# afermg/aliby

Hardware: AMD Instinct MI355X
Metric: FOV tiles/sec (whole node) (higher is better)
Workload: dtype u16 pixels, f64 feature accumulators, f32 dynamics, bfloat16 U-Net

## Files before the change

aliby_amd/_lib.py:

```python

from __future__ import annotations

import ctypes as C
import os
import threading
from pathlib import Path

import numpy as np

_HERE = Path(__file__).resolve().parent
LIB_PATH = Path(os.environ["ALIBY_HIP_LIB"]) if os.environ.get("ALIBY_HIP_LIB") else _HERE / "libaliby_hip.so"

OK, ERR_INVALID, ERR_OVERFLOW, ERR_HIP, ERR_TOO_LARGE, ERR_UNSUPPORTED = range(6)
U16, F32 = 0, 1
U8W = 4
U64, F64 = 2, 3
RED_MAX, RED_ADD, RED_DIV = 0, 1, 2


class AlibyHipError(RuntimeError):
    pass


class aliby_object(C.Structure):
# ... 90 lines not shown
    "aliby_nn_nhwc_to_nchw_f32": (_i, [_vp, _vp, _i, _i, _i, _i, _i, _vp, _vp, _vp]),
    "aliby_nn_tiles_to_nhwc8_bf16": (_i, [_vp, _vp, _i, _i, _i, _i, _vp, _vp, _vp, _vp, _vp]),
    "aliby_masks_workspace_bytes": (_sz, [_i, _i, _i]),
    "aliby_masks_from_flows": (_i, [_vp, _vp, _vp, _i, _i, _i, _i, C.c_float, C.c_float, _i, C.c_float, _vp, _sz,
                                    _vp, _vp, _vp, _vp]),
    "aliby_masks3d_workspace_bytes": (_sz, [_i, _i, _i, _i]),
    "aliby_masks_from_flows_3d": (_i, [_vp, _vp, _vp, _i, _i, _i, _i, _i, C.c_float, _i, C.c_float, _vp, _sz, _vp, _vp, _vp, _vp]),
    "aliby_features_intensity": (_i, [_vp, _vp, _vp, _i, _i, _i, _i, _i, _i, _vp, _i, _i, _i, _vp, _i, _i, _vp]),
    "aliby_features_sizeshape": (_i, [_vp, _vp, _i, _i, _i, _vp, _i, _i, _i, _i, _vp, _i, _i, _vp]),
    "aliby_features_feret": (_i, [_vp, _vp, _i, _i, _i, _vp, _i, _i, _vp, _i, _i, _vp]),
    "aliby_object_mec": (_i, [_vp, _vp, _i, _i, _i, _vp, _i, _i, _vp, _vp]),
    "aliby_features_zernike": (_i, [_vp, _vp, _vp, _i, _i, _i, _i, _i, _i, _vp, _i, _vp, _i, _vp, _i, _i, _vp]),
    "aliby_features_radial_zernikes_multi": (_i, [_vp, _vp, _vp, _i, _i, _i, _i, _i, _vp, _vp, _i, _vp, _i, _vp, _vp, _i, _vp]),
    "aliby_features_texture": (_i, [_vp, _vp, _vp, _i, _i, _i, _i, _i, _i, _vp, _i, _i, _i, _i, _i, _i, _vp, _i, _i, _vp]),
    "aliby_radial_geometry": (_i, [_vp, _vp, _i, _i, _i, _vp, _i, _i, _i, _i, _vp, _vp]),
    "aliby_features_radial_distribution": (_i, [_vp, _vp, _vp, _vp, _i, _i, _i, _i, _i, _i, _vp, _i, _i, _vp, _i, _i, _vp]),
    "aliby_features_cell_ratio": (_i, [_vp, _vp, _vp, _i, _i, _i, _i, _i, _i, _i, _vp, _i, _i, _vp, _vp]),
    "aliby_features_trap_background": (_i, [_vp, _vp, _vp, _i, _i, _i, _i, _i, _i, _vp, _vp]),
    "aliby_granularity_workspace_bytes": (_sz, [_i, _i, _i, _i, C.c_double, C.c_double]),
    "aliby_features_granularity": (_i, [_vp, _vp, _vp, _i, _i, _i, _i, _i, _i, _vp, _i, C.c_double, C.c_double, _i, _i, _i,
                                        _vp, _sz, _vp, _i, _i, _vp]),
    "aliby_radial_geometry_unscaled": (_i, [_vp, _vp, _i, _i, _i, _vp, _i, _i, _i, _i, C.c_double, _vp, _vp]),
    "aliby_features_radial_distribution_rings": (_i, [_vp, _vp, _vp, _vp, _i, _i, _i, _i, _i, _i, _vp, _i, _i, _i, _vp, _i, _i, _vp]),
    "aliby_features_cell": (_i, [_vp, _vp, _vp, _i, _i, _i, _i, _i, _i, _vp, _i, _i, _i, _i, _vp, _i, _i, _vp]),
    "aliby_features_coloc": (_i, [_vp, _vp, _vp, _i, _i, _i, _i, _i, _i, _i, _vp, _i, _i, _vp, _i, _i, _i, _i, _i,
                                  C.c_double, C.c_double, _vp, _vp, _vp]),
    "aliby_labels_apply_lut": (_i, [_vp, _vp, _i, _i, _i, _vp, _vp, _vp, _vp]),
    "aliby_features_intensity3d": (_i, [_vp, _vp, _vp, _i, _i, _i, _i, _i, _i, _vp, _vp, _i, _i, _vp]),
    "aliby_features_sizeshape3d": (_i, [_vp, _vp, _i, _i, _i, _i, _vp, _vp, _vp, _i, _i, _vp]),
    "aliby_coloc3d_lds_voxels": (_i, []),
    "aliby_features_coloc3d": (_i, [_vp, _vp, _vp, _i, _i, _i, _i, _i, _i, _vp, _i, _vp, _vp, _i, _i, _i, _i, _i, _i, _i,
                                    C.c_double, C.c_double, _vp]),
    "aliby_texture3d_lds_voxels": (_i, []),
    "aliby_features_texture3d": (_i, [_vp, _vp, _vp, _i, _i, _i, _i, _i, _i, _i, _vp, _i, _i, _vp, _i, _i, _vp]),
    "aliby_parquet_write": (_i, [C.c_char_p, _vp, _i, _vp, _i, _vp, _vp, _i]),
    "aliby_npz_write": (_i, [C.c_char_p, _vp, _i, _i]),
    "aliby_host_codecs": (_i, [C.POINTER(_i), C.POINTER(_i)]),
    "aliby_host_copy": (_i, [_vp, _vp, _sz, _i]),
    "aliby_object_ranks": (_i, [_vp, _vp, _vp, _i, _i, _i, _i, _i, _i, _vp, _i, _i, _vp, _vp, _vp]),
}

_lib = None


def exported_symbols() -> list[str]:
    return sorted(_SIGNATURES)


def load() -> C.CDLL:
    global _lib
    if _lib is not None:
        return _lib
    if not LIB_PATH.exists():
        raise AlibyHipError(
            f"{LIB_PATH} is missing: build it with `python -c 'import __graft_entry__ as g; g.build()'` "
            "(make -C aliby_amd/csrc). There is no CPU fallback for the HIP path."
        )
    try:
        import torch
    except Exception:
        pass
    lib = C.CDLL(str(LIB_PATH), mode=getattr(os, "RTLD_NOW", 2))
# ... 80 lines not shown
```

aliby_amd/csrc/feat_coloc.hip:

```cpp
#include "common.h"
#include "coloc_stats.h"

typedef unsigned short u16;

struct ColocArgs {
  const u16* labels;
  const void* planes;
  int F, C, Y, X, ch0, ch1;
  const aliby_object* tab;
  int n_obj;
  int cap;
  unsigned char* gscratch;
  double* out;
  int ld;
  int col_pearson, col_manders, col_rwc, col_costes;
  double thr;
  double scale_max;
  const unsigned int* ranks;
  const int* rmax;
};

struct PlaneRanks {
  const unsigned int* rk1;
  const unsigned int* rk2;
// ... 273 lines not shown
        if (lane == 0) {
          const double d1 = FA ? c4[0] : 0.0, d2 = SA ? c4[1] : 0.0;
          out[col_costes] = CA ? c4[2] / d1 : 0.0;
          out[col_costes + 1] = CA ? c4[3] / d2 : 0.0;
        }
      }
    }
  }
}


struct RankArgs {
  const u16* labels;
  const void* planes;
  int F, C, Y, X, channel;
  const aliby_object* tab;
  int n_obj, cap;
  unsigned char* gscratch;
  unsigned int* ranks;
  int* rmax;
};

template <typename T, bool GLOBAL>
__global__ __launch_bounds__(256) void k_ranks(RankArgs a) {
  extern __shared__ __align__(16) unsigned char lds_raw[];
  __shared__ int wsum[4];
  __shared__ int part[256];
  unsigned char* ws = GLOBAL ? (a.gscratch + (size_t)blockIdx.x * (size_t)a.cap * 16) : lds_raw;
  float* vals = reinterpret_cast<float*>(ws);
  float* S = vals + a.cap;
  int* P = reinterpret_cast<int*>(S + a.cap);
  int* pix = P + a.cap;
  const int tid = threadIdx.x;
  const size_t plane = (size_t)a.Y * a.X;
  for (int oi = blockIdx.x; oi < a.n_obj; oi += gridDim.x) {
    const aliby_object o = a.tab[oi];
    if (o.area <= 0) { if (tid == 0) a.rmax[(size_t)oi * a.C + a.channel] = 0; continue; }
    const u16* lab = a.labels + (size_t)o.tile * plane;
    const T* px = reinterpret_cast<const T*>(a.planes) + ((size_t)o.tile * a.C + a.channel) * plane;
    unsigned int* rk = a.ranks + ((size_t)o.tile * a.C + a.channel) * plane;
    const int h = o.y1 - o.y0, w = o.x1 - o.x0, npix = h * w;
    const u16 L = (u16)o.label;
    __syncthreads();
    int base = 0;
    for (int i0 = 0; i0 < npix; i0 += blockDim.x) {
      const int i = i0 + tid;
      bool in = false;
      size_t idx = 0;
      if (i < npix) { idx = (size_t)(o.y0 + i / w) * a.X + (o.x0 + i % w); in = lab[idx] == L; }
      const int pos = block_compact_slot(in, base, wsum);
      if (in) { vals[pos] = px_load<T>(px, idx); pix[pos] = (int)idx; }
    }
    __syncthreads();
    const int N = base;
    bool done = false;
    if (sizeof(T) == 2 && !GLOBAL) {
      int lo = INT_MAX, hi = 0;
      for (int j = tid; j < N; j += blockDim.x) { const int v = (int)vals[j]; lo = min(lo, v); hi = max(hi, v); }
      const int vmin = block_min_i32(lo, part), vmax = block_max_i32(hi, part);
      const int w0 = vmin >> 5, nw = (vmax >> 5) - w0 + 1;
      if (nw <= a.cap) {
        unsigned int* bits = reinterpret_cast<unsigned int*>(S);
        __syncthreads();
        for (int i = tid; i < nw; i += blockDim.x) bits[i] = 0u;
        __syncthreads();
        for (int j = tid; j < N; j += blockDim.x) { const int v = (int)vals[j]; atomicOr(&bits[(v >> 5) - w0], 1u << (v & 31)); }
        __syncthreads();
        for (int i = tid; i < nw; i += blockDim.x) P[i] = __popc(bits[i]);
        __syncthreads();
        block_inclusive_scan(P, nw, part);
        for (int j = tid; j < N; j += blockDim.x) {
          const int v = (int)vals[j], wi = (v >> 5) - w0;
          const unsigned int below = bits[wi] & ((1u << (v & 31)) - 1u);
          rk[pix[j]] = (unsigned int)(P[wi] - __popc(bits[wi]) + __popc(below));
        }
        if (tid == 0) a.rmax[(size_t)oi * a.C + a.channel] = P[nw - 1] - 1;
        done = true;
      }
    }
    if (done) { __syncthreads(); continue; }
    const int n2 = next_pow2(N);
    for (int i = tid; i < n2; i += blockDim.x) S[i] = (i < N) ? vals[i] : INFINITY;
    block_bitonic_sort(S, n2);
    for (int i = tid; i < N; i += blockDim.x) P[i] = (i > 0 && S[i] != S[i - 1]) ? 1 : 0;
    __syncthreads();
    block_inclusive_scan(P, N, part);
    for (int j = tid; j < N; j += blockDim.x) {
      const float v = vals[j];
      int lo = 0, hi = N;
      while (lo < hi) { const int mid = (lo + hi) >> 1; if (S[mid] < v) lo = mid + 1; else hi = mid; }
      rk[pix[j]] = (unsigned int)P[lo];
    }
    if (tid == 0) a.rmax[(size_t)oi * a.C + a.channel] = P[N - 1];
    __syncthreads();
  }
}

extern "C" int aliby_object_ranks(aliby_ctx* ctx, const uint16_t* labels, const void* planes, int dtype, int F, int C,
                                  int Y, int X, int channel, const aliby_object* table_dev, int n_obj, int max_area,
                                  uint32_t* ranks_dev, int32_t* rmax_dev, void* stream) {
  ARG_CHECK(ctx != nullptr, "ctx is NULL");
  if (n_obj == 0) return ALIBY_OK;
  ARG_CHECK(labels && planes && table_dev && ranks_dev && rmax_dev, "NULL argument");
  ARG_CHECK(dtype == ALIBY_U16 || dtype == ALIBY_F32, "dtype must be ALIBY_U16 or ALIBY_F32");
  ARG_CHECK(channel >= 0 && channel < C, "channel out of range");
  ARG_CHECK((size_t)Y * X < (size_t)INT_MAX, "plane too large");
  RankArgs a;
  a.labels = labels; a.planes = planes; a.F = F; a.C = C; a.Y = Y; a.X = X; a.channel = channel; a.tab = table_dev;
  a.n_obj = n_obj; a.ranks = ranks_dev; a.rmax = rmax_dev;
  int cap = 64;
  while (cap < max_area) cap <<= 1;
  a.cap = cap;
  hipStream_t s = as_stream(stream);
  const size_t need = (size_t)cap * 16;
  if (need <= 96 * 1024) {
    a.gscratch = nullptr;
    dim3 grid(n_obj), block(aliby_pick_block(max_area));
    if (dtype == ALIBY_U16) {
      if (need > 32 * 1024) HIP_TRY(hipFuncSetAttribute((const void*)k_ranks<u16, false>, hipFuncAttributeMaxDynamicSharedMemorySize, (int)need));
      hipLaunchKernelGGL((k_ranks<u16, false>), grid, block, need, s, a);
    } else {
      if (need > 32 * 1024) HIP_TRY(hipFuncSetAttribute((const void*)k_ranks<float, false>, hipFuncAttributeMaxDynamicSharedMemorySize, (int)need));
      hipLaunchKernelGGL((k_ranks<float, false>), grid, block, need, s, a);
    }
  } else {
    const int g = n_obj < 512 ? n_obj : 512;
    int rc = aliby_ensure_scratch(ctx, (size_t)g * need);
    if (rc) return rc;
    a.gscratch = (unsigned char*)ctx->scratch;
    dim3 grid(g), block(256);
    if (dtype == ALIBY_U16) hipLaunchKernelGGL((k_ranks<u16, true>), grid, block, 0, s, a);
    else hipLaunchKernelGGL((k_ranks<float, true>), grid, block, 0, s, a);
  }
  KERNEL_CHECK();
  return ALIBY_OK;
}

extern "C" int aliby_features_coloc(aliby_ctx* ctx, const uint16_t* labels, const void* planes, int dtype,
                                    int F, int C, int Y, int X, int ch0, int ch1,
                                    const aliby_object* table_dev, int n_obj, int max_area,
                                    double* out, int ld, int col_pearson, int col_manders, int col_rwc,
                                    int col_costes, double thr_percent, double costes_scale_max,
                                    const uint32_t* ranks_dev, const int32_t* rmax_dev, void* stream) {
  ARG_CHECK(ctx != nullptr, "ctx is NULL");
  if (n_obj == 0) return ALIBY_OK;
  ARG_CHECK(labels && planes && table_dev && out, "NULL argument");
  ARG_CHECK(dtype == ALIBY_U16 || dtype == ALIBY_F32, "dtype must be ALIBY_U16 or ALIBY_F32");
  ARG_CHECK(ch0 >= 0 && ch0 < C && ch1 >= 0 && ch1 < C, "channel out of range");
  ARG_CHECK(F > 0 && Y > 0 && X > 0 && max_area >= 0, "bad shape");
  const int cols[4] = {col_pearson, col_manders, col_rwc, col_costes};
  for (int k = 0; k < 4; ++k) ARG_CHECK(cols[k] < 0 || cols[k] + 2 <= ld, "columns exceed row stride");
  ColocArgs a;
  a.labels = labels; a.planes = planes; a.F = F; a.C = C; a.Y = Y; a.X = X; a.ch0 = ch0; a.ch1 = ch1;
  a.tab = table_dev; a.n_obj = n_obj; a.out = out; a.ld = ld;
  a.col_pearson = col_pearson; a.col_manders = col_manders; a.col_rwc = col_rwc; a.col_costes = col_costes;
  a.thr = thr_percent; a.scale_max = costes_scale_max;
  a.ranks = ranks_dev; a.rmax = rmax_dev;
  ARG_CHECK(col_rwc < 0 || (ranks_dev && rmax_dev), "rwc needs the rank planes (aliby_object_ranks)");
// ... 86 lines not shown
```

aliby_amd/csrc/feat_radial.hip:

```cpp
#include "common.h"

typedef unsigned short u16;

#define RD_MAXBINS 16
#define RD_INF 0xFFFFu

struct RadialGeoArgs {
  const u16* labels;
  int F, Y, X;
  const aliby_object* tab;
  int n_obj;
  size_t cap_cells;
  unsigned char* gscratch;
  int bin_count;
  double max_radius;
  unsigned char* binmap;
};

__device__ __forceinline__ double path_cost(unsigned int w) {
  return (double)(w & 0xFFFFu) * 0.70710678118654752440 + (double)(w >> 16) * 1.0;
}

template <bool GLOBAL>
__global__ __launch_bounds__(256) void k_radial_geometry(RadialGeoArgs a) {
// ... 164 lines not shown
    if (tid < a.nout) {
      double T_ = 0, N_ = 0;
      for (int b = 0; b <= nb; ++b) { T_ += tot[b]; N_ += (double)cnt[b]; }
      const double fd = tot[tid] / T_;
      const double fb = (double)cnt[tid] / N_;
      double mean = 0;
      int nw = 0;
      double m8[8];
      for (int k = 0; k < 8; ++k)
        if (wcnt[tid][k] > 0) { m8[nw] = wsum[tid][k] / (double)wcnt[tid][k]; mean += m8[nw]; ++nw; }
      double cv = 0.0;
      if (nw > 0) {
        mean /= (double)nw;
        double var = 0;
        for (int k = 0; k < nw; ++k) var += (m8[k] - mean) * (m8[k] - mean);
        cv = sqrt(var / (double)nw) / mean;
      }
      out[tid] = fd;
      out[a.nout + tid] = fd / (fb + 2.220446049250313e-16);
      out[2 * a.nout + tid] = cv;
    }
    __syncthreads();
  }
}

extern "C" {

int aliby_radial_geometry(aliby_ctx* ctx, const uint16_t* labels, int F, int Y, int X,
                          const aliby_object* table_dev, int n_obj, int max_h, int max_w, int bin_count,
                          uint8_t* binmap_dev, void* stream) {
  return aliby_radial_geometry_unscaled(ctx, labels, F, Y, X, table_dev, n_obj, max_h, max_w, bin_count, 0.0, binmap_dev, stream);
}

int aliby_radial_geometry_unscaled(aliby_ctx* ctx, const uint16_t* labels, int F, int Y, int X,
                                   const aliby_object* table_dev, int n_obj, int max_h, int max_w, int bin_count,
                                   double maximum_radius, uint8_t* binmap_dev, void* stream) {
  ARG_CHECK(ctx != nullptr, "ctx is NULL");
  if (n_obj == 0) return ALIBY_OK;
  ARG_CHECK(labels && table_dev && binmap_dev, "NULL argument");
  ARG_CHECK(F > 0 && Y > 0 && X > 0 && max_h >= 0 && max_w >= 0, "bad shape");
  ARG_CHECK(bin_count >= 1 && bin_count < RD_MAXBINS, "1 <= bin_count < 16");
  ARG_CHECK(max_h + max_w < 16000, "object too large for 16-bit path counters");
  RadialGeoArgs a;
  a.labels = labels; a.F = F; a.Y = Y; a.X = X; a.tab = table_dev; a.n_obj = n_obj; a.bin_count = bin_count;
  a.max_radius = maximum_radius;
  a.binmap = binmap_dev;
// ... 28 lines not shown
                                             const void* planes, int dtype, int F, int C, int Y, int X,
                                             int channel, const aliby_object* table_dev, int n_obj,
                                             int bin_count, int rings_out, double* out, int ld, int col0, void* stream) {
  ARG_CHECK(ctx != nullptr, "ctx is NULL");
  ARG_CHECK(rings_out == bin_count || rings_out == bin_count + 1, "rings_out is bin_count (scaled) or bin_count + 1 (with the overflow ring)");
  if (n_obj == 0) return ALIBY_OK;
  ARG_CHECK(labels && binmap_dev && planes && table_dev && out, "NULL argument");
  ARG_CHECK(dtype == ALIBY_U16 || dtype == ALIBY_F32, "dtype must be ALIBY_U16 or ALIBY_F32");
  ARG_CHECK(channel >= 0 && channel < C, "channel out of range");
  ARG_CHECK(bin_count >= 1 && bin_count < RD_MAXBINS, "1 <= bin_count < 16");
  ARG_CHECK(col0 >= 0 && col0 + 3 * rings_out <= ld, "columns exceed row stride");
  RadialStatArgs a;
  a.labels = labels; a.binmap = binmap_dev; a.planes = planes; a.F = F; a.C = C; a.Y = Y; a.X = X;
  a.channel = channel; a.tab = table_dev; a.n_obj = n_obj; a.bin_count = bin_count;
  a.nout = rings_out;
  a.out = out; a.ld = ld; a.col0 = col0;
  hipStream_t s = as_stream(stream);
  if (dtype == ALIBY_U16) hipLaunchKernelGGL((k_radial_stats<u16>), dim3(n_obj), dim3(256), 0, s, a);
  else hipLaunchKernelGGL((k_radial_stats<float>), dim3(n_obj), dim3(256), 0, s, a);
  KERNEL_CHECK();
  return ALIBY_OK;
}

}
```

aliby_amd/extraction/engine.py:

```python

from __future__ import annotations

import ctypes as C
from dataclasses import dataclass

import numpy as np
import torch

from aliby_amd import _lib
from aliby_amd.extraction import features as feat


def _stream_ptr() -> int:
    return torch.cuda.current_stream().cuda_stream


def _ptr(t) -> int:
    if t is None:
        return 0
    if isinstance(t, torch.Tensor):
        return t.data_ptr()
    if isinstance(t, np.ndarray):
        return t.ctypes.data
    raise TypeError(type(t))
# ... 474 lines not shown
        with self.timed("radial_geometry"):
            _lib.check(self.lib.aliby_radial_geometry_unscaled(
                self.ctx.handle, _ptr(labels), F, Y, X, _ptr(table.dev), table.n_obj, table.max_h, table.max_w, int(bin_count),
                0.0 if maximum_radius is None else float(maximum_radius), _ptr(binmap), _stream_ptr()))
        cache[key] = binmap
        return binmap

    def radial_distribution(self, labels, planes, dtype, channel, table: ObjectTable, out, col0, bin_count=4,
                            scaled=True, maximum_radius=100):
        if not scaled and not maximum_radius > 0:
            raise ValueError("radial_distribution(scaled=False) needs maximum_radius > 0")
        F, Cn, Y, X = planes.shape
        binmap = self.radial_geometry(labels, table, bin_count, None if scaled else maximum_radius)
        rings = bin_count if scaled else bin_count + 1
        with self.timed("radial_distribution"):
            _lib.check(
                self.lib.aliby_features_radial_distribution_rings(
                    self.ctx.handle, _ptr(labels), _ptr(binmap), _ptr(planes), _kdt(dtype), F, Cn, Y, X, int(channel),
                    _ptr(table.dev), table.n_obj, int(bin_count), rings, _ptr(out), out.stride(0), col0, _stream_ptr(),
                )
            )
        return 3 * rings

    def granularity(self, labels, planes, dtype, channel, table: ObjectTable, out, col0, subsample_size=0.25,
                    image_sample_size=0.25, element_size=10, granular_spectrum_length=16, image_mask="frame", mask_order=1):
        if image_mask not in ("frame", "objects"):
            raise ValueError(f"image_mask must be 'frame' or 'objects', got {image_mask!r}")
        if image_mask == "objects" and int(mask_order) != 1:
            raise NotImplementedError("granularity(image_mask='objects') is built for mask_order=1 (bilinear) only")
        F, Cn, Y, X = planes.shape
        L = int(granular_spectrum_length)
        need = int(self.lib.aliby_granularity_workspace_bytes(F, Y, X, table.n_obj, float(subsample_size), float(image_sample_size)))
        work = torch.empty((need + 7) // 8, dtype=torch.float64, device=labels.device)
        with self.timed("granularity"):
            _lib.check(
                self.lib.aliby_features_granularity(
                    self.ctx.handle, _ptr(labels), _ptr(planes), _kdt(dtype), F, Cn, Y, X, int(channel), _ptr(table.dev), table.n_obj,
                    float(subsample_size), float(image_sample_size), int(element_size), L, 1 if image_mask == "objects" else 0,
                    _ptr(work), work.numel() * 8, _ptr(out), out.stride(0) if table.n_obj else max(L + col0, 1), col0, _stream_ptr(),
                )
            )
        return L

    CELL_COLUMNS = ("area", "centroid_x", "centroid_y", "conical_volume", "eccentricity", "spherical_volume", "volume",
                    "min_ax", "maj_ax", "mean", "median", "std", "total", "total_squared", "max2p5pc", "max5px_median",
                    "moment_of_inertia")
# ... 16 lines not shown
        F, Cn, Y, X = planes.shape
        out = torch.full((max(table.n_obj, 1),), float("nan"), dtype=torch.float64, device=labels.device)
        with self.timed("cell_metrics"):
            _lib.check(self.lib.aliby_features_cell_ratio(self.ctx.handle, _ptr(labels), _ptr(planes), _kdt(dtype), F, Cn, Y, X, int(ch0), int(ch1),
                                                          _ptr(table.dev), table.n_obj, table.max_area, _ptr(out), _stream_ptr()))
        return out[: table.n_obj]

    def trap_background(self, labels, planes, dtype, channel) -> torch.Tensor:
        F, Cn, Y, X = planes.shape
        out = torch.empty((F, 2), dtype=torch.float64, device=labels.device)
        with self.timed("trap_background"):
            _lib.check(self.lib.aliby_features_trap_background(self.ctx.handle, _ptr(labels), _ptr(planes), _kdt(dtype), F, Cn, Y, X, int(channel),
                                                               _ptr(out), _stream_ptr()))
        return out

    def rank_planes(self, labels, planes, dtype, table: ObjectTable, channels):
        F, Cn, Y, X = planes.shape
        key = ("ranks", planes.data_ptr())
        cache = table.__dict__.setdefault("_ranks", {})
        if key not in cache:
            cache[key] = dict(ranks=torch.empty((F, Cn, Y, X), dtype=torch.int32, device=planes.device),
                              rmax=torch.zeros((max(table.n_obj, 1), Cn), dtype=torch.int32, device=planes.device), done=set())
        e = cache[key]
        for ch in channels:
            if ch in e["done"]:
                continue
            with self.timed("ranks"):
                _lib.check(self.lib.aliby_object_ranks(self.ctx.handle, _ptr(labels), _ptr(planes), _kdt(dtype), F, Cn, Y, X, int(ch),
                                                       _ptr(table.dev), table.n_obj, table.max_area, _ptr(e["ranks"]),
                                                       _ptr(e["rmax"]), _stream_ptr()))
            e["done"].add(ch)
        return e["ranks"], e["rmax"]

    def coloc_pairs(self, labels, planes, dtype, pairs, table: ObjectTable, out, thr=15.0, scale_max=255.0) -> bool:
        F, Cn, Y, X = planes.shape
        chans = sorted({c for (pair, _) in pairs for c in pair})
        any_rwc = any(cols.get("rwc") is not None for _, cols in pairs)
        cap = 64
        while cap < table.max_area:
            cap <<= 1
        if len(pairs) > 28 or len(chans) > 8 or len(chans) * cap * 4 * (2 if any_rwc else 1) > 144 * 1024:
            return False
        ranks = rmax = None
        if any_rwc:
            ranks, rmax = self.rank_planes(labels, planes, dtype, table, tuple(chans))
        c = lambda cols, k: -1 if cols.get(k) is None else int(cols[k])
        spec = np.asarray([[ch0, ch1, c(cols, "pearson"), c(cols, "manders_fold"), c(cols, "rwc"), c(cols, "costes")]
                           for (ch0, ch1), cols in pairs], dtype=np.int32)
        with self.timed("coloc"):
            _lib.check(
                self.lib.aliby_features_coloc_pairs(
                    self.ctx.handle, _ptr(labels), _ptr(planes), _kdt(dtype), F, Cn, Y, X, spec.ctypes.data, len(pairs), _ptr(table.dev),
                    table.n_obj, table.max_area, _ptr(out), out.stride(0), float(thr), float(scale_max),
                    _ptr(ranks) if ranks is not None else 0, _ptr(rmax) if rmax is not None else 0, _stream_ptr(),
# ... 21 lines not shown
```

aliby_amd/extraction/families.py:

```python

from __future__ import annotations

import torch

from aliby_amd import _lib
from aliby_amd.extraction import features as feat
from aliby_amd.extraction.engine import _ptr, _stream_ptr

_RED = {"max": _lib.RED_MAX, "add": _lib.RED_ADD, "div": _lib.RED_DIV}


class PlaneCache:

    def __init__(self, eng, planes):
        self.eng = eng
        self.tensor, self.dtype = planes
        if self.tensor.ndim != 5:
            raise Exception(f"pixels must be [F,C,Z,Y,X], got {tuple(self.tensor.shape)}")
        self._cache = {}

    def get(self, red_z):
        if red_z in self._cache:
            return self._cache[red_z]
        if red_z not in _RED:
# ... 203 lines not shown
        for inst, reg, kw, col0, _ in specs:
            (ch0, ch1), red_ch, red_z, metric = inst[0], inst[1], inst[2], inst[3]
            if red_ch != "None":
                raise NotImplementedError(
                    "channel-combining multi instructions (extract.py:227-235) are not built; "
                    "the builder only emits red_ch='None' (pipe_builder.py:33-43)"
                )
            thr = float(kw.get("thr", 15.0)) if metric in ("manders_fold", "rwc") else None
            scale_max = float(kw.get("scale_max", 255.0)) if metric == "costes" else None
            groups.setdefault(((ch0, ch1), red_z), []).append((metric, col0, thr, scale_max))
        split = {}
        for key, entries in groups.items():
            thrs = sorted({t for _, _, t, _ in entries if t is not None})
            scale_max = next((sm for _, _, _, sm in entries if sm is not None), 255.0)
            if len(thrs) <= 1:
                split[(key, 0)] = dict(cols={m: c for m, c, _, _ in entries}, thr=thrs[0] if thrs else 15.0, scale_max=scale_max)
            else:
                for k, t in enumerate(thrs):
                    cols = {m: c for m, c, tt, _ in entries if tt == t or (tt is None and k == 0)}
                    split[(key, k)] = dict(cols=cols, thr=t, scale_max=scale_max)
        groups = {(pair_z, k): g for (pair_z, k), g in split.items()}
        if cache is None:
            raise Exception("pixels are required for colocalisation instructions")
        for (((ch0, ch1), red_z), _k), g in groups.items():
            plane, dt = cache.get(red_z)
            if "rwc" in g["cols"]:
                eng.rank_planes(labels, plane, dt, table, (ch0, ch1))
        import os

        batches = {}
        for (((ch0, ch1), red_z), _k), g in groups.items():
            batches.setdefault((red_z, g["thr"], g["scale_max"]), []).append(((ch0, ch1), g["cols"]))
        left = []
        for (red_z, thr, scale_max), pairs in batches.items():
            plane, dt = cache.get(red_z)
            if os.environ.get("ALIBY_COLOC_PAIRS", "1") == "0" or len(pairs) < 2 or not eng.coloc_pairs(
                    labels, plane, dt, pairs, table, out, thr=thr, scale_max=scale_max):
                left.extend((pair, red_z, cols, thr, scale_max) for pair, cols in pairs)
        if left:
            fan.fork()
            for (ch0, ch1), red_z, cols, thr, scale_max in left:
                plane, dt = cache.get(red_z)
                with fan.next_stream():
                    eng.coloc(labels, plane, dt, ch0, ch1, table, out, cols, thr=thr, scale_max=scale_max)
            fan.join()
        return out, blocks

    for inst, reg, kw, col0, ncols in specs:
        metric = inst[-1]
        if inst[0] != "None" and reg["needs_pixels"] and cache is not None and inst[1] in _RED:
            cache.get(inst[1])
        if metric in ("zernike", "radial_zernikes") and table.n_obj:
            eng.mec(labels, table)
        if metric == "radial_distribution" and table.n_obj:
            eng.radial_geometry(labels, table, kw.get("bin_count", 4), None if kw.get("scaled", True) else kw.get("maximum_radius", 100))
    fan.fork()
    done = {}
    copies, after = [], []
    zern_groups = {}
    sizeshape_col0 = next((c0 for inst, reg, kw, c0, _ in specs if inst[-1] == "sizeshape"), None)
    cell_cache = {}
    for spec in specs:
        inst, reg, kw, col0, ncols = spec
        ch, red_z, metric = inst[0], inst[1], inst[-1]
        if reg.get("cell"):
            after.append(spec)
            continue
        if ch == "None" or not reg["needs_pixels"]:
            if ch != "None" and cache is not None:
                cache.get(red_z)
            key = (metric, tuple(sorted(kw.items())))
            if metric == "feret" and sizeshape_col0 is not None:
                ss = feat.sizeshape_names()
                for j, name in enumerate(feat.feret_names()):
                    copies.append((col0 + j, sizeshape_col0 + ss.index(name), 1))
            elif key in done:
                copies.append((col0, done[key], ncols))
            else:
                with fan.next_stream():
                    reg["launch"](eng, labels, table, None, 0, None, out, col0, kw)
                done[key] = col0
        else:
            if cache is None:
                raise Exception("pixels are required for this instruction")
            plane, dt = cache.get(red_z)
            if metric == "radial_zernikes" and hasattr(eng, "radial_zernikes_multi") and table.n_obj:
                zern_groups.setdefault(red_z, []).append((ch, col0))
                continue
            with fan.next_stream():
                reg["launch"](eng, labels, table, plane, dt, ch, out, col0, kw)
    for red_z, members in zern_groups.items():
        plane, dt = cache.get(red_z)
        with fan.next_stream():
            eng.radial_zernikes_multi(labels, plane, dt, [c for c, _ in members], table, out, [c0 for _, c0 in members])
    fan.join()
    for col0, src, ncols in copies:
        out[:, col0 : col0 + ncols] = out[:, src : src + ncols]
    for inst, reg, kw, col0, ncols in after:
        ch, red_z = inst[0], inst[1]
        extra = {"cell_cache": cell_cache}
        if ch == "None" or not reg["needs_pixels"]:
            if ch != "None" and cache is not None:
                cache.get(red_z)
            reg["launch"](eng, labels, table, None, 0, None, out, col0, kw, **extra)
        else:
            if cache is None:
                raise Exception("pixels are required for this instruction")
            plane, dt = cache.get(red_z)
            reg["launch"](eng, labels, table, plane, dt, ch, out, col0, kw, **extra)
    return out, blocks
```

include/aliby_hip.h:

```cpp
#ifndef ALIBY_HIP_H
#define ALIBY_HIP_H

#include <stddef.h>
#include <stdint.h>

#ifdef __cplusplus
extern "C" {
#endif

#define ALIBY_ABI_VERSION 1

enum {
  ALIBY_OK = 0,
  ALIBY_ERR_INVALID = 1,
  ALIBY_ERR_OVERFLOW = 2,
  ALIBY_ERR_HIP = 3,
  ALIBY_ERR_TOO_LARGE = 4,
  ALIBY_ERR_UNSUPPORTED = 5
};

enum { ALIBY_U16 = 0, ALIBY_F32 = 1,
       ALIBY_U64 = 2, ALIBY_F64 = 3 ,
       ALIBY_U8W = 4  };

// ... 159 lines not shown
int aliby_features_radial_zernikes_multi(aliby_ctx* ctx, const uint16_t* labels, const void* planes, int dtype, int F, int C, int Y,
                                         int X, const int* channels, const int* col0s, int n_channels, const aliby_object* table_dev,
                                         int n_obj, const double* mec_dev, double* out, int ld, void* stream);

int aliby_features_texture(aliby_ctx* ctx, const uint16_t* labels, const void* planes, int dtype,
                           int F, int C, int Y, int X, int channel, const aliby_object* table_dev,
                           int n_obj, int max_h, int max_w, int max_area, int scale, int gray_levels,
                           double* out, int ld, int col0, void* stream);

int aliby_radial_geometry(aliby_ctx* ctx, const uint16_t* labels, int F, int Y, int X,
                          const aliby_object* table_dev, int n_obj, int max_h, int max_w, int bin_count,
                          uint8_t* binmap_dev, void* stream);
int aliby_features_radial_distribution(aliby_ctx* ctx, const uint16_t* labels, const uint8_t* binmap_dev,
                                       const void* planes, int dtype, int F, int C, int Y, int X,
                                       int channel, const aliby_object* table_dev, int n_obj,
                                       int bin_count, double* out, int ld, int col0, void* stream);
int aliby_radial_geometry_unscaled(aliby_ctx* ctx, const uint16_t* labels, int F, int Y, int X,
                                   const aliby_object* table_dev, int n_obj, int max_h, int max_w, int bin_count,
                                   double maximum_radius, uint8_t* binmap_dev, void* stream);
int aliby_features_radial_distribution_rings(aliby_ctx* ctx, const uint16_t* labels, const uint8_t* binmap_dev,
                                             const void* planes, int dtype, int F, int C, int Y, int X,
                                             int channel, const aliby_object* table_dev, int n_obj,
                                             int bin_count, int rings_out, double* out, int ld, int col0, void* stream);

int aliby_features_cell(aliby_ctx* ctx, const uint16_t* labels, const void* planes, int dtype, int F, int C,
                        int Y, int X, int channel, const aliby_object* table_dev, int n_obj, int max_h,
                        int max_w, int max_area, double* out, int ld, int col0, void* stream);

int aliby_features_cell_ratio(aliby_ctx* ctx, const uint16_t* labels, const void* planes, int dtype, int F, int C, int Y,
                              int X, int channel0, int channel1, const aliby_object* table_dev, int n_obj, int max_area,
                              double* out, void* stream);
int aliby_features_trap_background(aliby_ctx* ctx, const uint16_t* labels, const void* planes, int dtype, int F, int C,
                                   int Y, int X, int channel, double* out, void* stream);

size_t aliby_granularity_workspace_bytes(int F, int Y, int X, int n_obj, double subsample_size, double image_sample_size);
int aliby_features_granularity(aliby_ctx* ctx, const uint16_t* labels, const void* planes, int dtype, int F, int C, int Y,
                               int X, int channel, const aliby_object* table_dev, int n_obj, double subsample_size,
                               double image_sample_size, int element_size, int spectrum_length, int image_mask_objects,
                               void* workspace, size_t workspace_bytes, double* out, int ld, int col0, void* stream);

int aliby_features_coloc(aliby_ctx* ctx, const uint16_t* labels, const void* planes, int dtype,
                         int F, int C, int Y, int X, int ch0, int ch1,
                         const aliby_object* table_dev, int n_obj, int max_area,
                         double* out, int ld, int col_pearson, int col_manders, int col_rwc,
                         int col_costes, double thr_percent, double costes_scale_max,
                         const uint32_t* ranks_dev, const int32_t* rmax_dev, void* stream);
int aliby_features_coloc_pairs(aliby_ctx* ctx, const uint16_t* labels, const void* planes, int dtype, int F, int C,
                               int Y, int X, const int32_t* pairs_host, int n_pairs, const aliby_object* table_dev,
                               int n_obj, int max_area, double* out, int ld, double thr_percent,
                               double costes_scale_max, const uint32_t* ranks_dev, const int32_t* rmax_dev,
                               void* stream);
int aliby_object_ranks(aliby_ctx* ctx, const uint16_t* labels, const void* planes, int dtype, int F, int C,
                       int Y, int X, int channel, const aliby_object* table_dev, int n_obj, int max_area,
                       uint32_t* ranks_dev, int32_t* rmax_dev, void* stream);

int aliby_tiff_probe(const char* path, int64_t* info, char* description, int description_len);
int aliby_ingest_tiff_planes(aliby_ctx* ctx, const char* const* paths, const int32_t* pages, int n, int width,
                             int height, int bytes_per_sample, void* dst, size_t plane_stride, int dst_is_device,
                             int n_threads, void* stream);
int aliby_ingest_inflate(int codec, const void* src, size_t src_bytes, void* dst, size_t dst_bytes,
                         size_t* out_bytes);

int aliby_trap_gauss1d(aliby_ctx* ctx, const double* in, double* out, int H, int W, int axis,
                       const double* weights_dev, int radius, int truncate, void* stream);
int aliby_trap_warp(aliby_ctx* ctx, const double* in, int H, int W, double* out, int OH, int OW,
                    const double* matrix6_host, int mode, double cval, void* stream);
int aliby_trap_entropy(aliby_ctx* ctx, const uint8_t* in, int H, int W, int radius, double* out, void* stream);
int aliby_trap_morph(aliby_ctx* ctx, const uint8_t* in, uint8_t* out, int H, int W, int lo, int hi, int is_max,
                     void* stream);
int aliby_trap_label(aliby_ctx* ctx, const uint8_t* bw, int H, int W, int32_t* labels, void* stream);
int aliby_trap_region_sums(aliby_ctx* ctx, const int32_t* labels, int H, int W, uint64_t* sums, void* stream);
int aliby_trap_match_template(aliby_ctx* ctx, const double* padded, int PH, int PW, const double* templ, int th,
                              int tw, double* out, int H, int W, double t_mean, double t_ssd, void* stream);
int aliby_trap_maxfilter1d(aliby_ctx* ctx, const double* in, double* out, int H, int W, int axis, int radius,
                           void* stream);

int aliby_labels_apply_lut(aliby_ctx* ctx, const uint16_t* labels_in, int T, int Y, int X, const int32_t* offsets_host,
// ... 42 lines not shown
```

Measured before the change: 612.4.

## Batch rank and radial-distribution kernels across channels in single launches

Adds multi-channel variants of the per-object rank kernel and the radial-distribution stats kernel. Each block compacts an object's mask pixels once and reuses that compaction, or the binmap scan, for up to five channels. Previously this was redone in a separate launch per channel. The Python layer groups channels by reduction plane and settings and dispatches them in chunks. This saves kernel launches and repeated label/binmap reads, at the cost of more LDS use per block for the radial kernel and more template instantiations.

```diff
diff --git a/aliby_amd/_lib.py b/aliby_amd/_lib.py
--- a/aliby_amd/_lib.py
+++ b/aliby_amd/_lib.py
@@ -136,6 +136,7 @@
                                         _vp, _sz, _vp, _i, _i, _vp]),
     "aliby_radial_geometry_unscaled": (_i, [_vp, _vp, _i, _i, _i, _vp, _i, _i, _i, _i, C.c_double, _vp, _vp]),
     "aliby_features_radial_distribution_rings": (_i, [_vp, _vp, _vp, _vp, _i, _i, _i, _i, _i, _i, _vp, _i, _i, _i, _vp, _i, _i, _vp]),
+    "aliby_features_radial_distribution_multi": (_i, [_vp, _vp, _vp, _vp, _i, _i, _i, _i, _i, _vp, _vp, _i, _vp, _i, _i, _i, _vp, _i, _vp]),
     "aliby_features_cell": (_i, [_vp, _vp, _vp, _i, _i, _i, _i, _i, _i, _vp, _i, _i, _i, _i, _vp, _i, _i, _vp]),
     "aliby_features_coloc": (_i, [_vp, _vp, _vp, _i, _i, _i, _i, _i, _i, _i, _vp, _i, _i, _vp, _i, _i, _i, _i, _i,
                                   C.c_double, C.c_double, _vp, _vp, _vp]),
@@ -152,6 +153,7 @@
     "aliby_host_codecs": (_i, [C.POINTER(_i), C.POINTER(_i)]),
     "aliby_host_copy": (_i, [_vp, _vp, _sz, _i]),
     "aliby_object_ranks": (_i, [_vp, _vp, _vp, _i, _i, _i, _i, _i, _i, _vp, _i, _i, _vp, _vp, _vp]),
+    "aliby_object_ranks_multi": (_i, [_vp, _vp, _vp, _i, _i, _i, _i, _i, _vp, _i, _vp, _i, _i, _vp, _vp, _vp]),
 }
 
 _lib = None
diff --git a/aliby_amd/csrc/feat_coloc.hip b/aliby_amd/csrc/feat_coloc.hip
--- a/aliby_amd/csrc/feat_coloc.hip
+++ b/aliby_amd/csrc/feat_coloc.hip
@@ -319,6 +319,51 @@
 };
 
 template <typename T, bool GLOBAL>
+__device__ __forceinline__ void ranks_of_staged(const float* vals, float* S, int* P, const int* pix, int N, int cap, unsigned int* rk,
+                                                int* rmax, int* part) {
+  const int tid = threadIdx.x;
+  if (sizeof(T) == 2 && !GLOBAL) {
+    int lo = INT_MAX, hi = 0;
+    for (int j = tid; j < N; j += blockDim.x) { const int v = (int)vals[j]; lo = min(lo, v); hi = max(hi, v); }
+    const int vmin = block_min_i32(lo, part), vmax = block_max_i32(hi, part);
+    const int w0 = vmin >> 5, nw = (vmax >> 5) - w0 + 1;
+    if (nw <= cap) {
+      unsigned int* bits = reinterpret_cast<unsigned int*>(S);
+      __syncthreads();
+      for (int i = tid; i < nw; i += blockDim.x) bits[i] = 0u;
+      __syncthreads();
+      for (int j = tid; j < N; j += blockDim.x) { const int v = (int)vals[j]; atomicOr(&bits[(v >> 5) - w0], 1u << (v & 31)); }
+      __syncthreads();
+      for (int i = tid; i < nw; i += blockDim.x) P[i] = __popc(bits[i]);
+      __syncthreads();
+      block_inclusive_scan(P, nw, part);
+      for (int j = tid; j < N; j += blockDim.x) {
+        const int v = (int)vals[j], wi = (v >> 5) - w0;
+        const unsigned int below = bits[wi] & ((1u << (v & 31)) - 1u);
+        rk[pix[j]] = (unsigned int)(P[wi] - __popc(bits[wi]) + __popc(below));
+      }
+      if (tid == 0) *rmax = P[nw - 1] - 1;
+      __syncthreads();
+      return;
+    }
+  }
+  const int n2 = next_pow2(N);
+  for (int i = tid; i < n2; i += blockDim.x) S[i] = (i < N) ? vals[i] : INFINITY;
+  block_bitonic_sort(S, n2);
+  for (int i = tid; i < N; i += blockDim.x) P[i] = (i > 0 && S[i] != S[i - 1]) ? 1 : 0;
+  __syncthreads();
+  block_inclusive_scan(P, N, part);
+  for (int j = tid; j < N; j += blockDim.x) {
+    const float v = vals[j];
+    int lo = 0, hi = N;
+    while (lo < hi) { const int mid = (lo + hi) >> 1; if (S[mid] < v) lo = mid + 1; else hi = mid; }
+    rk[pix[j]] = (unsigned int)P[lo];
+  }
+  if (tid == 0) *rmax = P[N - 1];
+  __syncthreads();
+}
+
+template <typename T, bool GLOBAL>
 __global__ __launch_bounds__(256) void k_ranks(RankArgs a) {
   extern __shared__ __align__(16) unsigned char lds_raw[];
   __shared__ int wsum[4];
@@ -349,48 +394,84 @@
       if (in) { vals[pos] = px_load<T>(px, idx); pix[pos] = (int)idx; }
     }
     __syncthreads();
-    const int N = base;
-    bool done = false;
-    if (sizeof(T) == 2 && !GLOBAL) {
-      int lo = INT_MAX, hi = 0;
-      for (int j = tid; j < N; j += blockDim.x) { const int v = (int)vals[j]; lo = min(lo, v); hi = max(hi, v); }
-      const int vmin = block_min_i32(lo, part), vmax = block_max_i32(hi, part);
-      const int w0 = vmin >> 5, nw = (vmax >> 5) - w0 + 1;
-      if (nw <= a.cap) {
-        unsigned int* bits = reinterpret_cast<unsigned int*>(S);
-        __syncthreads();
-        for (int i = tid; i < nw; i += blockDim.x) bits[i] = 0u;
-        __syncthreads();
-        for (int j = tid; j < N; j += blockDim.x) { const int v = (int)vals[j]; atomicOr(&bits[(v >> 5) - w0], 1u << (v & 31)); }
-        __syncthreads();
-        for (int i = tid; i < nw; i += blockDim.x) P[i] = __popc(bits[i]);
-        __syncthreads();
-        block_inclusive_scan(P, nw, part);
-        for (int j = tid; j < N; j += blockDim.x) {
-          const int v = (int)vals[j], wi = (v >> 5) - w0;
-          const unsigned int below = bits[wi] & ((1u << (v & 31)) - 1u);
-          rk[pix[j]] = (unsigned int)(P[wi] - __popc(bits[wi]) + __popc(below));
-        }
-        if (tid == 0) a.rmax[(size_t)oi * a.C + a.channel] = P[nw - 1] - 1;
-        done = true;
-      }
-    }
-    if (done) { __syncthreads(); continue; }
-    const int n2 = next_pow2(N);
-    for (int i = tid; i < n2; i += blockDim.x) S[i] = (i < N) ? vals[i] : INFINITY;
-    block_bitonic_sort(S, n2);
-    for (int i = tid; i < N; i += blockDim.x) P[i] = (i > 0 && S[i] != S[i - 1]) ? 1 : 0;
-    __syncthreads();
-    block_inclusive_scan(P, N, part);
-    for (int j = tid; j < N; j += blockDim.x) {
-      const float v = vals[j];
-      int lo = 0, hi = N;
-      while (lo < hi) { const int mid = (lo + hi) >> 1; if (S[mid] < v) lo = mid + 1; else hi = mid; }
-      rk[pix[j]] = (unsigned int)P[lo];
-    }
-    if (tid == 0) a.rmax[(size_t)oi * a.C + a.channel] = P[N - 1];
-    __syncthreads();
-  }
+    ranks_of_staged<T, GLOBAL>(vals, S, P, pix, base, a.cap, rk, &a.rmax[(size_t)oi * a.C + a.channel], part);
+  }
+}
+
+struct RankMultiArgs {
+  const u16* labels;
+  const void* planes;
+  int F, C, Y, X;
+  int channel[ALIBY_MULTI_MAXCH];
+  const aliby_object* tab;
+  int n_obj, cap;
+  unsigned char* gscratch;
+  unsigned int* ranks;
+  int* rmax;
+};
+
+template <typename T, bool GLOBAL, int NCH>
+__global__ __launch_bounds__(256) void k_ranks_multi(RankMultiArgs a) {
+  extern __shared__ __align__(16) unsigned char lds_raw[];
+  __shared__ int wsum[4];
+  __shared__ int part[256];
+  unsigned char* ws = GLOBAL ? (a.gscratch + (size_t)blockIdx.x * (size_t)a.cap * 16) : lds_raw;
+  float* vals = reinterpret_cast<float*>(ws);
+  float* S = vals + a.cap;
+  int* P = reinterpret_cast<int*>(S + a.cap);
+  int* pix = P + a.cap;
+  const int tid = threadIdx.x;
+  const size_t plane = (size_t)a.Y * a.X;
+  for (int oi = blockIdx.x; oi < a.n_obj; oi += gridDim.x) {
+    const aliby_object o = a.tab[oi];
+    if (o.area <= 0) {
+      if (tid < NCH) a.rmax[(size_t)oi * a.C + a.channel[tid]] = 0;
+      continue;
+    }
+    const u16* lab = a.labels + (size_t)o.tile * plane;
+    const int h = o.y1 - o.y0, w = o.x1 - o.x0, npix = h * w;
+    const u16 L = (u16)o.label;
+    __syncthreads();
+    int base = 0;
+    for (int i0 = 0; i0 < npix; i0 += blockDim.x) {
+      const int i = i0 + tid;
+      bool in = false;
+      size_t idx = 0;
+      if (i < npix) { idx = (size_t)(o.y0 + i / w) * a.X + (o.x0 + i % w); in = lab[idx] == L; }
+      const int pos = block_compact_slot(in, base, wsum);
+      if (in) pix[pos] = (int)idx;
+    }
+    __syncthreads();
+#pragma unroll 1
+    for (int c = 0; c < NCH; ++c) {
+      const int ch = a.channel[c];
+      const T* px = reinterpret_cast<const T*>(a.planes) + ((size_t)o.tile * a.C + ch) * plane;
+      unsigned int* rk = a.ranks + ((size_t)o.tile * a.C + ch) * plane;
+      for (int j = tid; j < base; j += blockDim.x) vals[j] = px_load<T>(px, (size_t)pix[j]);
+      __syncthreads();
+      ranks_of_staged<T, GLOBAL>(vals, S, P, pix, base, a.cap, rk, &a.rmax[(size_t)oi * a.C + ch], part);
+    }
+  }
+}
+
+template <typename T, bool GLOBAL>
+static int launch_ranks_multi(const RankMultiArgs& a, int nch, dim3 grid, dim3 block, size_t lds, hipStream_t s) {
+#define RANKS_MULTI_CASE(N)                                                                                                    \
+  case N:                                                                                                                      \
+    if (lds > 32 * 1024)                                                                                                       \
+      HIP_TRY(hipFuncSetAttribute((const void*)k_ranks_multi<T, GLOBAL, N>, hipFuncAttributeMaxDynamicSharedMemorySize, (int)lds)); \
+    hipLaunchKernelGGL((k_ranks_multi<T, GLOBAL, N>), grid, block, lds, s, a);                                                 \
+    break;
+  switch (nch) {
+    RANKS_MULTI_CASE(2)
+    RANKS_MULTI_CASE(3)
+    RANKS_MULTI_CASE(4)
+    RANKS_MULTI_CASE(5)
+    default: aliby_set_error("ranks: 2 to 5 channels per launch, got %d", nch); return ALIBY_ERR_INVALID;
+  }
+#undef RANKS_MULTI_CASE
+  KERNEL_CHECK();
+  return ALIBY_OK;
 }
 
 extern "C" int aliby_object_ranks(aliby_ctx* ctx, const uint16_t* labels, const void* planes, int dtype, int F, int C,
@@ -431,6 +512,45 @@
   }
   KERNEL_CHECK();
   return ALIBY_OK;
+}
+
+extern "C" int aliby_object_ranks_multi(aliby_ctx* ctx, const uint16_t* labels, const void* planes, int dtype, int F, int C, int Y,
+                                        int X, const int* channels, int n_channels, const aliby_object* table_dev, int n_obj,
+                                        int max_area, uint32_t* ranks_dev, int32_t* rmax_dev, void* stream) {
+  ARG_CHECK(ctx != nullptr, "ctx is NULL");
+  if (n_obj == 0) return ALIBY_OK;
+  ARG_CHECK(labels && planes && table_dev && ranks_dev && rmax_dev && channels, "NULL argument");
+  ARG_CHECK(dtype == ALIBY_U16 || dtype == ALIBY_F32, "dtype must be ALIBY_U16 or ALIBY_F32");
+  ARG_CHECK(n_channels >= 2 && n_channels <= ALIBY_MULTI_MAXCH, "2 <= n_channels <= 5");
+  ARG_CHECK(F > 0 && Y > 0 && X > 0 && max_area >= 0, "bad shape");
+  ARG_CHECK((size_t)Y * X < (size_t)INT_MAX, "plane too large");
+  RankMultiArgs a;
+  a.labels = labels; a.planes = planes; a.F = F; a.C = C; a.Y = Y; a.X = X; a.tab = table_dev;
+  for (int i = 0; i < ALIBY_MULTI_MAXCH; ++i) a.channel[i] = 0;
+  for (int i = 0; i < n_channels; ++i) {
+    ARG_CHECK(channels[i] >= 0 && channels[i] < C, "channel out of range");
+    for (int j = 0; j < i; ++j) ARG_CHECK(channels[j] != channels[i], "channels must be distinct");
+    a.channel[i] = channels[i];
+  }
+  a.n_obj = n_obj; a.ranks = ranks_dev; a.rmax = rmax_dev;
+  int cap = 64;
+  while (cap < max_area) cap <<= 1;
+  a.cap = cap;
+  hipStream_t s = as_stream(stream);
+  const size_t need = (size_t)cap * 16;
+  if (need <= 96 * 1024) {
+    a.gscratch = nullptr;
+    dim3 grid(n_obj), block(aliby_pick_block(max_area));
+    return dtype == ALIBY_U16 ? launch_ranks_multi<u16, false>(a, n_channels, grid, block, need, s)
+                              : launch_ranks_multi<float, false>(a, n_channels, grid, block, need, s);
+  }
+  const int g = n_obj < 512 ? n_obj : 512;
+  int rc = aliby_ensure_scratch(ctx, (size_t)g * need);
+  if (rc) return rc;
+  a.gscratch = (unsigned char*)ctx->scratch;
+  dim3 grid(g), block(256);
+  return dtype == ALIBY_U16 ? launch_ranks_multi<u16, true>(a, n_channels, grid, block, 0, s)
+                            : launch_ranks_multi<float, true>(a, n_channels, grid, block, 0, s);
 }
 
 extern "C" int aliby_features_coloc(aliby_ctx* ctx, const uint16_t* labels, const void* planes, int dtype,
diff --git a/aliby_amd/csrc/feat_radial.hip b/aliby_amd/csrc/feat_radial.hip
--- a/aliby_amd/csrc/feat_radial.hip
+++ b/aliby_amd/csrc/feat_radial.hip
@@ -210,6 +210,109 @@
     }
     __syncthreads();
   }
+}
+
+struct RadialStatMultiArgs {
+  const u16* labels;
+  const unsigned char* binmap;
+  const void* planes;
+  int F, C, Y, X;
+  int channel[ALIBY_MULTI_MAXCH], col0[ALIBY_MULTI_MAXCH];
+  const aliby_object* tab;
+  int n_obj, bin_count;
+  int nout;
+  double* out;
+  int ld;
+};
+
+template <typename T, int NCH>
+__global__ __launch_bounds__(256) void k_radial_stats_multi(RadialStatMultiArgs a) {
+  __shared__ double tot[NCH][RD_MAXBINS + 1];
+  __shared__ int cnt[RD_MAXBINS + 1];
+  __shared__ double wsum[NCH][RD_MAXBINS + 1][8];
+  __shared__ int wcnt[RD_MAXBINS + 1][8];
+  const int tid = threadIdx.x;
+  const size_t plane = (size_t)a.Y * a.X;
+  const int nb = a.bin_count;
+  for (int oi = blockIdx.x; oi < a.n_obj; oi += gridDim.x) {
+    const aliby_object o = a.tab[oi];
+    if (o.area <= 0) {
+      for (int k = tid; k < 3 * a.nout * NCH; k += blockDim.x) {
+        const int ch = k / (3 * a.nout);
+        a.out[(size_t)oi * a.ld + a.col0[ch] + (k - ch * 3 * a.nout)] = NAN;
+      }
+      continue;
+    }
+    __syncthreads();
+    for (int k = tid; k < NCH * (RD_MAXBINS + 1) * 8; k += blockDim.x) (&wsum[0][0][0])[k] = 0;
+    for (int k = tid; k < (RD_MAXBINS + 1) * 8; k += blockDim.x) (&wcnt[0][0])[k] = 0;
+    for (int k = tid; k < NCH * (RD_MAXBINS + 1); k += blockDim.x) (&tot[0][0])[k] = 0;
+    for (int k = tid; k <= RD_MAXBINS; k += blockDim.x) cnt[k] = 0;
+    __syncthreads();
+    const u16* lab = a.labels + (size_t)o.tile * plane;
+    const unsigned char* bm = a.binmap + (size_t)o.tile * plane;
+    const T* px[NCH];
+#pragma unroll
+    for (int ch = 0; ch < NCH; ++ch) px[ch] = reinterpret_cast<const T*>(a.planes) + ((size_t)o.tile * a.C + a.channel[ch]) * plane;
+    const int h = o.y1 - o.y0, w = o.x1 - o.x0;
+    const u16 L = (u16)o.label;
+    for (int i = tid; i < h * w; i += blockDim.x) {
+      const size_t idx = (size_t)(o.y0 + i / w) * a.X + (o.x0 + i % w);
+      if (lab[idx] != L) continue;
+      const int code = bm[idx];
+      if (!(code & 0x80)) continue;
+      const int bin = code & 15, wedge = (code >> 4) & 7;
+      double v[NCH];
+#pragma unroll
+      for (int ch = 0; ch < NCH; ++ch) v[ch] = (double)px_load<T>(px[ch], idx);
+      atomicAdd(&cnt[bin], 1);
+      atomicAdd(&wcnt[bin][wedge], 1);
+#pragma unroll
+      for (int ch = 0; ch < NCH; ++ch) {
+        atomicAdd(&tot[ch][bin], v[ch]);
+        atomicAdd(&wsum[ch][bin][wedge], v[ch]);
+      }
+    }
+    __syncthreads();
+    if (tid < a.nout * NCH) {
+      const int ch = tid / a.nout, ring = tid - ch * a.nout;
+      double* out = a.out + (size_t)oi * a.ld + a.col0[ch];
+      double T_ = 0, N_ = 0;
+      for (int b = 0; b <= nb; ++b) { T_ += tot[ch][b]; N_ += (double)cnt[b]; }
+      const double fd = tot[ch][ring] / T_;
+      const double fb = (double)cnt[ring] / N_;
+      double mean = 0;
+      int nw = 0;
+      double m8[8];
+      for (int k = 0; k < 8; ++k)
+        if (wcnt[ring][k] > 0) { m8[nw] = wsum[ch][ring][k] / (double)wcnt[ring][k]; mean += m8[nw]; ++nw; }
+      double cv = 0.0;
+      if (nw > 0) {
+        mean /= (double)nw;
+        double var = 0;
+        for (int k = 0; k < nw; ++k) var += (m8[k] - mean) * (m8[k] - mean);
+        cv = sqrt(var / (double)nw) / mean;
+      }
+      out[ring] = fd;
+      out[a.nout + ring] = fd / (fb + 2.220446049250313e-16);
+      out[2 * a.nout + ring] = cv;
+    }
+    __syncthreads();
+  }
+}
+
+template <typename T>
+static int launch_radial_stats_multi(const RadialStatMultiArgs& a, int nch, hipStream_t s) {
+  dim3 grid(a.n_obj), block(256);
+  switch (nch) {
+    case 2: hipLaunchKernelGGL((k_radial_stats_multi<T, 2>), grid, block, 0, s, a); break;
+    case 3: hipLaunchKernelGGL((k_radial_stats_multi<T, 3>), grid, block, 0, s, a); break;
+    case 4: hipLaunchKernelGGL((k_radial_stats_multi<T, 4>), grid, block, 0, s, a); break;
+    case 5: hipLaunchKernelGGL((k_radial_stats_multi<T, 5>), grid, block, 0, s, a); break;
+    default: aliby_set_error("radial_distribution: 2 to 5 channels per launch, got %d", nch); return ALIBY_ERR_INVALID;
+  }
+  KERNEL_CHECK();
+  return ALIBY_OK;
 }
 
 extern "C" {
@@ -284,4 +387,29 @@
   return ALIBY_OK;
 }
 
-}
+int aliby_features_radial_distribution_multi(aliby_ctx* ctx, const uint16_t* labels, const uint8_t* binmap_dev, const void* planes,
+                                             int dtype, int F, int C, int Y, int X, const int* channels, const int* col0s,
+                                             int n_channels, const aliby_object* table_dev, int n_obj, int bin_count,
+                                             int rings_out, double* out, int ld, void* stream) {
+  ARG_CHECK(ctx != nullptr, "ctx is NULL");
+  ARG_CHECK(rings_out == bin_count || rings_out == bin_count + 1, "rings_out is bin_count (scaled) or bin_count + 1 (with the overflow ring)");
+  if (n_obj == 0) return ALIBY_OK;
+  ARG_CHECK(labels && binmap_dev && planes && table_dev && out && channels && col0s, "NULL argument");
+  ARG_CHECK(dtype == ALIBY_U16 || dtype == ALIBY_F32, "dtype must be ALIBY_U16 or ALIBY_F32");
+  ARG_CHECK(n_channels >= 2 && n_channels <= ALIBY_MULTI_MAXCH, "2 <= n_channels <= 5");
+  ARG_CHECK(bin_count >= 1 && bin_count < RD_MAXBINS, "1 <= bin_count < 16");
+  RadialStatMultiArgs a;
+  a.labels = labels; a.binmap = binmap_dev; a.planes = planes; a.F = F; a.C = C; a.Y = Y; a.X = X;
+  for (int i = 0; i < ALIBY_MULTI_MAXCH; ++i) { a.channel[i] = 0; a.col0[i] = 0; }
+  for (int i = 0; i < n_channels; ++i) {
+    ARG_CHECK(channels[i] >= 0 && channels[i] < C, "channel out of range");
+    ARG_CHECK(col0s[i] >= 0 && col0s[i] + 3 * rings_out <= ld, "columns exceed row stride");
+    a.channel[i] = channels[i];
+    a.col0[i] = col0s[i];
+  }
+  a.tab = table_dev; a.n_obj = n_obj; a.bin_count = bin_count; a.nout = rings_out; a.out = out; a.ld = ld;
+  hipStream_t s = as_stream(stream);
+  return dtype == ALIBY_U16 ? launch_radial_stats_multi<u16>(a, n_channels, s) : launch_radial_stats_multi<float>(a, n_channels, s);
+}
+
+}
diff --git a/aliby_amd/extraction/engine.py b/aliby_amd/extraction/engine.py
--- a/aliby_amd/extraction/engine.py
+++ b/aliby_amd/extraction/engine.py
@@ -520,6 +520,38 @@
             )
         return 3 * rings
 
+    @staticmethod
+    def _multi_chunks(n_total: int):
+        k = 0
+        while k < n_total:
+            n = min(5, n_total - k)
+            if n_total - k - n == 1:
+                n -= 1
+            yield k, n
+            k += n
+
+    def radial_distribution_multi(self, labels, planes, dtype, channels, table: ObjectTable, out, col0s, bin_count=4, scaled=True,
+                                  maximum_radius=100):
+        channels, col0s = list(map(int, channels)), list(map(int, col0s))
+        if len(channels) < 2:
+            for ch, c0 in zip(channels, col0s):
+                self.radial_distribution(labels, planes, dtype, ch, table, out, c0, bin_count=bin_count, scaled=scaled,
+                                         maximum_radius=maximum_radius)
+            return 3 * (bin_count if scaled else bin_count + 1)
+        if not scaled and not maximum_radius > 0:
+            raise ValueError("radial_distribution(scaled=False) needs maximum_radius > 0")
+        F, Cn, Y, X = planes.shape
+        binmap = self.radial_geometry(labels, table, bin_count, None if scaled else maximum_radius)
+        rings = bin_count if scaled else bin_count + 1
+        for k, n in self._multi_chunks(len(channels)):
+            ch = (C.c_int * n)(*channels[k : k + n])
+            c0 = (C.c_int * n)(*col0s[k : k + n])
+            with self.timed("radial_distribution"):
+                _lib.check(self.lib.aliby_features_radial_distribution_multi(
+                    self.ctx.handle, _ptr(labels), _ptr(binmap), _ptr(planes), _kdt(dtype), F, Cn, Y, X, ch, c0, n, _ptr(table.dev),
+                    table.n_obj, int(bin_count), rings, _ptr(out), out.stride(0), _stream_ptr()))
+        return 3 * rings
+
     def granularity(self, labels, planes, dtype, channel, table: ObjectTable, out, col0, subsample_size=0.25,
                     image_sample_size=0.25, element_size=10, granular_spectrum_length=16, image_mask="frame", mask_order=1):
         if image_mask not in ("frame", "objects"):
@@ -582,14 +614,23 @@
             cache[key] = dict(ranks=torch.empty((F, Cn, Y, X), dtype=torch.int32, device=planes.device),
                               rmax=torch.zeros((max(table.n_obj, 1), Cn), dtype=torch.int32, device=planes.device), done=set())
         e = cache[key]
+        todo = []
         for ch in channels:
-            if ch in e["done"]:
-                continue
+            if int(ch) not in e["done"] and int(ch) not in todo:
+                todo.append(int(ch))
+        if len(todo) == 1:
             with self.timed("ranks"):
-                _lib.check(self.lib.aliby_object_ranks(self.ctx.handle, _ptr(labels), _ptr(planes), _kdt(dtype), F, Cn, Y, X, int(ch),
+                _lib.check(self.lib.aliby_object_ranks(self.ctx.handle, _ptr(labels), _ptr(planes), _kdt(dtype), F, Cn, Y, X, todo[0],
                                                        _ptr(table.dev), table.n_obj, table.max_area, _ptr(e["ranks"]),
                                                        _ptr(e["rmax"]), _stream_ptr()))
-            e["done"].add(ch)
+        elif todo:
+            for k, n in self._multi_chunks(len(todo)):
+                chs = (C.c_int * n)(*todo[k : k + n])
+                with self.timed("ranks"):
+                    _lib.check(self.lib.aliby_object_ranks_multi(self.ctx.handle, _ptr(labels), _ptr(planes), _kdt(dtype), F, Cn, Y, X, chs, n,
+                                                                 _ptr(table.dev), table.n_obj, table.max_area, _ptr(e["ranks"]),
+                                                                 _ptr(e["rmax"]), _stream_ptr()))
+        e["done"].update(todo)
         return e["ranks"], e["rmax"]
 
     def coloc_pairs(self, labels, planes, dtype, pairs, table: ObjectTable, out, thr=15.0, scale_max=255.0) -> bool:
diff --git a/aliby_amd/extraction/families.py b/aliby_amd/extraction/families.py
--- a/aliby_amd/extraction/families.py
+++ b/aliby_amd/extraction/families.py
@@ -249,10 +249,14 @@
         groups = {(pair_z, k): g for (pair_z, k), g in split.items()}
         if cache is None:
             raise Exception("pixels are required for colocalisation instructions")
+        rank_channels = {}
         for (((ch0, ch1), red_z), _k), g in groups.items():
+            cache.get(red_z)
+            if "rwc" in g["cols"]:
+                rank_channels.setdefault(red_z, []).extend((ch0, ch1))
+        for red_z, chans in rank_channels.items():
             plane, dt = cache.get(red_z)
-            if "rwc" in g["cols"]:
-                eng.rank_planes(labels, plane, dt, table, (ch0, ch1))
+            eng.rank_planes(labels, plane, dt, table, tuple(dict.fromkeys(chans)))
         import os
 
         batches = {}
@@ -285,6 +289,7 @@
     done = {}
     copies, after = [], []
     zern_groups = {}
+    radial_groups = {}
     sizeshape_col0 = next((c0 for inst, reg, kw, c0, _ in specs if inst[-1] == "sizeshape"), None)
     cell_cache = {}
     for spec in specs:
@@ -314,12 +319,22 @@
             if metric == "radial_zernikes" and hasattr(eng, "radial_zernikes_multi") and table.n_obj:
                 zern_groups.setdefault(red_z, []).append((ch, col0))
                 continue
+            if metric == "radial_distribution" and hasattr(eng, "radial_distribution_multi") and table.n_obj:
+                radial_groups.setdefault((red_z, tuple(sorted(kw.items()))), []).append((ch, col0))
+                continue
             with fan.next_stream():
                 reg["launch"](eng, labels, table, plane, dt, ch, out, col0, kw)
     for red_z, members in zern_groups.items():
         plane, dt = cache.get(red_z)
         with fan.next_stream():
             eng.radial_zernikes_multi(labels, plane, dt, [c for c, _ in members], table, out, [c0 for _, c0 in members])
+    for (red_z, kw_items), members in radial_groups.items():
+        plane, dt = cache.get(red_z)
+        kw = dict(kw_items)
+        with fan.next_stream():
+            eng.radial_distribution_multi(labels, plane, dt, [c for c, _ in members], table, out, [c0 for _, c0 in members],
+                                          bin_count=kw.get("bin_count", 4), scaled=kw.get("scaled", True),
+                                          maximum_radius=kw.get("maximum_radius", 100))
     fan.join()
     for col0, src, ncols in copies:
         out[:, col0 : col0 + ncols] = out[:, src : src + ncols]
diff --git a/include/aliby_hip.h b/include/aliby_hip.h
--- a/include/aliby_hip.h
+++ b/include/aliby_hip.h
@@ -205,6 +205,11 @@
                                              const void* planes, int dtype, int F, int C, int Y, int X,
                                              int channel, const aliby_object* table_dev, int n_obj,
                                              int bin_count, int rings_out, double* out, int ld, int col0, void* stream);
+#define ALIBY_MULTI_MAXCH 5
+int aliby_features_radial_distribution_multi(aliby_ctx* ctx, const uint16_t* labels, const uint8_t* binmap_dev, const void* planes,
+                                             int dtype, int F, int C, int Y, int X, const int* channels, const int* col0s,
+                                             int n_channels, const aliby_object* table_dev, int n_obj, int bin_count,
+                                             int rings_out, double* out, int ld, void* stream);
 
 int aliby_features_cell(aliby_ctx* ctx, const uint16_t* labels, const void* planes, int dtype, int F, int C,
                         int Y, int X, int channel, const aliby_object* table_dev, int n_obj, int max_h,
@@ -236,6 +241,9 @@
 int aliby_object_ranks(aliby_ctx* ctx, const uint16_t* labels, const void* planes, int dtype, int F, int C,
                        int Y, int X, int channel, const aliby_object* table_dev, int n_obj, int max_area,
                        uint32_t* ranks_dev, int32_t* rmax_dev, void* stream);
+int aliby_object_ranks_multi(aliby_ctx* ctx, const uint16_t* labels, const void* planes, int dtype, int F, int C, int Y, int X,
+                             const int* channels, int n_channels, const aliby_object* table_dev, int n_obj, int max_area,
+                             uint32_t* ranks_dev, int32_t* rmax_dev, void* stream);
 
 int aliby_tiff_probe(const char* path, int64_t* info, char* description, int description_len);
 int aliby_ingest_tiff_planes(aliby_ctx* ctx, const char* const* paths, const int32_t* pages, int n, int width,
```

Result: no change. 614.4, median of 6 (+0.3%).
